# RaptorMai/online-continual-learning

Measured on NVIDIA H100. Metric: replay-step images/sec (ASER+SCR, ResNet18, CIFAR100), higher is better.
Workload: dtype f32

## Files before the change

online-continual-learning_b200/csrc/conv_tcp.cu:

```cuda
#include "conv.cuh"
#include "umma.cuh"

namespace b200ocl {
namespace {

constexpr int TP_THREADS = 32 * 13;
constexpr int TP_LOADER_WARP = 9;
constexpr int TP_PS_MAX = 3;
constexpr int TP_BS_MAX = 6;
constexpr int TP_CONSUMER_WARPS = 8;

using umma::mbar_expect_tx;
using umma::bulk_g2s;

struct TileGeom {
  int wp, pp;
  int tiles_m;
  int prow;
  int pbytes;
};
__host__ __device__ inline TileGeom tile_geom(int N, int H, int W) {
  TileGeom g;
  g.wp = W + 2;
  g.pp = (H + 2) * (W + 2);
  const long last = (long)(N - 1) * g.pp + (long)(H - 1) * g.wp + (W - 1);
  g.tiles_m = (int)(last / 128) + 1;
  g.prow = 128 + 2 * g.wp + 2;
  g.pbytes = (g.prow * 128 + 1023) / 1024 * 1024;
  return g;
}

template <int NT, int KS>
__device__ __forceinline__ void issue_tap(float (&d)[NT / 2], uint64_t dAh, uint64_t dAl, uint64_t dBh, uint64_t dBl) {
  umma::fence();
#pragma unroll
  for (int k = 0; k < KS; ++k) {
    const uint64_t adv = (uint64_t)(k * 2);
    umma::mma_tf32_ss<NT>(d, dAh + adv, dBh + adv, k > 0 ? 1u : 0u);
    umma::mma_tf32_ss<NT>(d, dAh + adv, dBl + adv, 1u);
    umma::mma_tf32_ss<NT>(d, dAl + adv, dBh + adv, 1u);
  }
  umma::commit();
  umma::wait<0>();
  umma::fence_regs(d);
}

template <int NT>
__global__ void __launch_bounds__(TP_THREADS, 1) conv_tcp_kernel(ConvArgs a) {
  constexpr int B_BLOCK = 2 * NT * 32;
  constexpr int R = NT / 2;
  extern __shared__ __align__(1024) unsigned char smem_raw[];
  unsigned char* patch0 = smem_raw;
  __shared__ __align__(8) uint64_t pfull[TP_PS_MAX], pempty[TP_PS_MAX], bfull[9], bempty[TP_BS_MAX];
  __shared__ int s_fail;
  __shared__ float s_coef[3 * 80];

  const int tid = threadIdx.x, warp = tid >> 5;
  const int bn = a.tp_bn;
  const int n0 = blockIdx.y * bn;
  const int slices = a.tp_slices;
  const TileGeom G = tile_geom(a.N, a.Hin, a.Win);
  const int PS = a.tp_ps, BS = a.tp_bs;
  float* sB = reinterpret_cast<float*>(smem_raw + (size_t)PS * 2 * G.pbytes);
  const bool resident = (slices == 1 && NT == 32);
  const int b_slots = resident ? 9 : BS;
  float* s_acc = sB + (size_t)b_slots * B_BLOCK;

  if (tid == 0) {
    for (int i = 0; i < TP_PS_MAX; ++i) {
      umma::mbar_init(&pfull[i], 128);
      umma::mbar_init(&pempty[i], TP_CONSUMER_WARPS);
    }
    for (int i = 0; i < 9; ++i) umma::mbar_init(&bfull[i], 1);
    for (int i = 0; i < TP_BS_MAX; ++i) umma::mbar_init(&bempty[i], TP_CONSUMER_WARPS);
    umma::fence_mbar_init();
    s_fail = 0;
  }
  __syncthreads();
  const float* wimg = a.w_tp + (size_t)blockIdx.y * slices * 9 * B_BLOCK;

  if (warp >= TP_LOADER_WARP) {
    const int lt = tid - 32 * TP_LOADER_WARP;
    int pc = 0;
    for (int tile = blockIdx.x; tile < a.tp_tiles; tile += gridDim.x) {
      for (int sl = 0; sl < slices; ++sl, ++pc) {
        const int ch_valid = min(32, a.CK - sl * 32);
        const int nch = 2 * ((ch_valid + 7) / 8);
        const int ch = lt & 7, r0 = lt >> 3;
        const int nrow = G.prow;
        const bool ch_live = ch < nch, ch_real = ch * 4 < ch_valid;
        float4 v[TP_LD_MAX];
        int img, yp, xp;
        {
          const int sp = tile * 128 + r0;
          img = sp / G.pp;
          const int rem = sp - img * G.pp;
          yp = rem / G.wp;
          xp = rem - yp * G.wp;
        }
        const int hp = a.Hin + 2;
#pragma unroll
        for (int i = 0; i < TP_LD_MAX; ++i) {
          v[i] = make_float4(0.f, 0.f, 0.f, 0.f);
          const int ri = r0 + 16 * i;
          if (ch_real && ri < nrow) {
            const int y = yp - 1, x = xp - 1;
            if (img < a.N && (unsigned)y < (unsigned)a.Hin && (unsigned)x < (unsigned)a.Win)
              v[i] = __ldg(reinterpret_cast<const float4*>(a.in + ((size_t)(img * a.Hin + y) * a.Win + x) * a.CK + sl * 32) + ch);
          }
          xp += 16;
          while (xp >= G.wp) {
            xp -= G.wp;
            if (++yp == hp) {
              yp = 0;
              ++img;
            }
          }
        }
        const int ps = pc % PS;
        if (!umma::mbar_wait(&pempty[ps], (uint32_t)(((pc / PS) & 1) ^ 1))) s_fail = 1;
        float* ph = reinterpret_cast<float*>(patch0 + (size_t)ps * 2 * G.pbytes);
        float* pl = ph + G.pbytes / 4;
        if (ch_live) {
#pragma unroll
          for (int i = 0; i < TP_LD_MAX; ++i) {
            const int ri = r0 + 16 * i;
            if (ri < nrow) {
              float4 h, l;
              umma::split_tf32(v[i].x, h.x, l.x); umma::split_tf32(v[i].y, h.y, l.y);
              umma::split_tf32(v[i].z, h.z, l.z); umma::split_tf32(v[i].w, h.w, l.w);
              const int off = umma::sw128_offset_f32(ri, ch);
              *reinterpret_cast<float4*>(ph + off) = h;
              *reinterpret_cast<float4*>(pl + off) = l;
            }
          }
        }
        umma::fence_proxy_async_smem();
        umma::mbar_arrive(&pfull[ps]);
      }
    }
  } else if (warp == TP_LOADER_WARP - 1) {
    const uint32_t bytes = (uint32_t)(B_BLOCK * sizeof(float));
    if (resident) {
      if (umma::elect_one_sync()) {
        for (int b = 0; b < 9; ++b) {
          mbar_expect_tx(&bfull[b], bytes);
          bulk_g2s(sB + (size_t)b * B_BLOCK, wimg + (size_t)b * B_BLOCK, bytes, &bfull[b]);
        }
      }
    } else {
      int q = 0;
      for (int tile = blockIdx.x; tile < a.tp_tiles; tile += gridDim.x)
        for (int sl = 0; sl < slices; ++sl)
          for (int tap = 0; tap < 9; ++tap, ++q) {
            const int bs = q % BS;
            if (!umma::mbar_wait(&bempty[bs], (uint32_t)(((q / BS) & 1) ^ 1))) s_fail = 1;
            if (umma::elect_one_sync()) {
              mbar_expect_tx(&bfull[bs], bytes);
              bulk_g2s(sB + (size_t)bs * B_BLOCK, wimg + (size_t)(sl * 9 + tap) * B_BLOCK, bytes, &bfull[bs]);
            }
            __syncwarp();
          }
    }
  } else {
    const int g = warp >> 2, wt = tid & 127;
    const int et = tid;
    const bool epi = tid < 128;
    const bool lane0 = (tid & 31) == 0;
    auto esync = []() { asm volatile("bar.sync 1, 128;\n" ::); };
    auto csync = []() { asm volatile("bar.sync 2, 256;\n" ::); };
    const uint64_t dA0 = umma::make_smem_desc_sw128(umma::smem_u32(patch0) + (uint32_t)(g * 64 * 128));
    const uint64_t dB0 = umma::make_smem_desc_sw128(umma::smem_u32(sB));
    const uint32_t A_LO = (uint32_t)G.pbytes >> 4;
    const uint32_t A_STAGE = (uint32_t)(2 * G.pbytes) >> 4;
    constexpr uint32_t B_LO = (NT * 128) >> 4;
    constexpr uint32_t B_SLOT = (B_BLOCK * 4) >> 4;
    if (epi && a.mode == CONV_EVAL) {
      for (int c = et; c < bn; c += 128) {
        const float inv = 1.0f / sqrtf(a.rvar[n0 + c] + a.eps);
        s_coef[c] = a.rmean[n0 + c];
        s_coef[80 + c] = inv * a.gamma[n0 + c];
        s_coef[160 + c] = a.beta[n0 + c];
      }
      esync();
    }
    int pc = 0, q = 0;
    bool b_ready = false;
    for (int tile = blockIdx.x; tile < a.tp_tiles; tile += gridDim.x) {
      float accf[R];
#pragma unroll
      for (int i = 0; i < R; ++i) accf[i] = 0.f;
      for (int sl = 0; sl < slices; ++sl, ++pc) {
        const int ps = pc % PS;
        const int ksteps = (min(32, a.CK - sl * 32) + 7) / 8;
        if (!umma::mbar_wait(&pfull[ps], (uint32_t)((pc / PS) & 1))) s_fail = 1;
        const uint64_t dAs = dA0 + (uint64_t)(ps * A_STAGE);
#pragma unroll 1
        for (int tap = 0; tap < 9; ++tap, ++q) {
          const int kh = tap / 3, kw = tap - 3 * kh;
          const int b = resident ? tap : q % BS;
          if (!(resident && b_ready))
            if (!umma::mbar_wait(&bfull[b], resident ? 0u : (uint32_t)((q / BS) & 1))) s_fail = 1;
          const uint64_t dAh = dAs + (uint64_t)((kh * G.wp + kw) * 8);
          const uint64_t dAl = dAh + A_LO;
          const uint64_t dBh = dB0 + (uint64_t)(b * B_SLOT);
          const uint64_t dBl = dBh + B_LO;
          float tmp[R];
          switch (ksteps) {
            case 1: issue_tap<NT, 1>(tmp, dAh, dAl, dBh, dBl); break;
            case 2: issue_tap<NT, 2>(tmp, dAh, dAl, dBh, dBl); break;
            case 3: issue_tap<NT, 3>(tmp, dAh, dAl, dBh, dBl); break;
            default: issue_tap<NT, 4>(tmp, dAh, dAl, dBh, dBl); break;
          }
#pragma unroll
          for (int i = 0; i < R; ++i) accf[i] += tmp[i];
          if (!resident && lane0) umma::mbar_arrive(&bempty[b]);
        }
        b_ready = true;
        if (lane0) umma::mbar_arrive(&pempty[ps]);
      }
      csync();
#pragma unroll
      for (int i = 0; i < R; ++i) s_acc[(64 * g + umma::frag_row(wt, i)) * (NT + 1) + umma::frag_col(wt, i)] = accf[i];
      csync();
      if (!epi) continue;
      const int sp = tile * 128 + et;
      const int img = sp / G.pp, rem = sp - img * G.pp;
      const int y = rem / G.wp, x = rem - y * G.wp;
      const bool valid = img < a.N && y < a.Hin && x < a.Win;
      const size_t m = ((size_t)img * a.Hin + y) * a.Win + x;
      float acc[NT], pre[NT];
#pragma unroll
      for (int c = 0; c < NT; ++c) {
        acc[c] = 0.f;
        pre[c] = 0.f;
      }
      {
        const float* src = nullptr;
        if (valid && a.mode == CONV_EVAL && a.residual) src = a.residual + m * a.CN + n0;
        if (valid && a.mode == CONV_ACCUM) src = a.out + m * a.CN + n0;
        if (src) {
#pragma unroll
          for (int c0 = 0; c0 < NT; c0 += 4) {
            if (c0 >= bn) break;
            const float4 v = *reinterpret_cast<const float4*>(src + c0);
            pre[c0] = v.x; pre[c0 + 1] = v.y; pre[c0 + 2] = v.z; pre[c0 + 3] = v.w;
          }
        }
      }
#pragma unroll
      for (int c = 0; c < NT; ++c) acc[c] = s_acc[et * (NT + 1) + c];
      if (a.mode == CONV_EVAL) {
        if (valid) {
          float* o = a.out + m * a.CN + n0;
#pragma unroll
          for (int c0 = 0; c0 < NT; c0 += 4) {
            if (c0 >= bn) break;
            float rr[4];
#pragma unroll
            for (int j = 0; j < 4; ++j) {
              rr[j] = (acc[c0 + j] - s_coef[c0 + j]) * s_coef[80 + c0 + j] + s_coef[160 + c0 + j];
              rr[j] += pre[c0 + j];
              if (a.relu) rr[j] = fmaxf(rr[j], 0.f);
            }
            *reinterpret_cast<float4*>(o + c0) = make_float4(rr[0], rr[1], rr[2], rr[3]);
          }
        }
      } else if (valid) {
        float* o = a.out + m * a.CN + n0;
#pragma unroll
        for (int c0 = 0; c0 < NT; c0 += 4) {
          if (c0 >= bn) break;
          *reinterpret_cast<float4*>(o + c0) = make_float4(acc[c0] + pre[c0], acc[c0 + 1] + pre[c0 + 1],
                                                           acc[c0 + 2] + pre[c0 + 2], acc[c0 + 3] + pre[c0 + 3]);
        }
      }
    }
  }
  __syncthreads();
  if (s_fail && tid == 0) a.out[(size_t)n0] = __int_as_float(0x7fc00000);
}

template <int NT>
size_t tcp_smem_bytes(const TileGeom& G, int slices, int ps, int bs) {
  const int b_slots = (slices == 1 && NT == 32) ? 9 : bs;
  return (size_t)ps * 2 * G.pbytes + (size_t)b_slots * 2 * NT * 32 * sizeof(float) +
         (size_t)128 * (NT + 1) * sizeof(float) + 1024;
}

template <int NT>
int launch_tcp(ConvArgs a, cudaStream_t stream) {
  const TileGeom G = tile_geom(a.N, a.Hin, a.Win);
  const size_t limit = 227 * 1024 - 4096
                       - (size_t)128 * (a.tp_bn + 1) * sizeof(float);
  a.tp_ps = 3; a.tp_bs = 6;
  if (tcp_smem_bytes<NT>(G, a.tp_slices, a.tp_ps, a.tp_bs) > limit) a.tp_bs = 4;
  if (tcp_smem_bytes<NT>(G, a.tp_slices, a.tp_ps, a.tp_bs) > limit) { a.tp_ps = 2; a.tp_bs = 6; }
  const size_t smem = tcp_smem_bytes<NT>(G, a.tp_slices, a.tp_ps, a.tp_bs);
  B200OCL_CUDA(raise_smem_limit<conv_tcp_kernel<NT>>(smem));
  a.tp_tiles = G.tiles_m;
  const int n_tiles = a.CN / a.tp_bn;
  int gx = sm_count() / n_tiles;
  if (gx < 1) gx = 1;
  if (gx > G.tiles_m) gx = G.tiles_m;
  const int rounds = (G.tiles_m + gx - 1) / gx;
  gx = (G.tiles_m + rounds - 1) / rounds;
  B200OCL_PROF("conv_tcp",
               2.0 * a.M * (double)a.CN * a.CK * 9.0, stream);
  conv_tcp_kernel<NT><<<dim3(gx, n_tiles), TP_THREADS, smem, stream>>>(a);
  B200OCL_LAUNCHED();
  return B200OCL_OK;
}

}

bool conv_tcp_eligible(const ConvArgs& a) {
  if (a.mode == CONV_TRAIN || !a.w_tp || a.transposed || a.CK % 4 != 0) return false;
  if (a.ks != 3 || a.pad != 1 || a.stride != 1 || a.Hout != a.Hin || a.Wout != a.Win) return false;
  if (!tcp_strip_fits(a.Win)) return false;
  if ((long)a.N * (a.Hin + 2) * (a.Win + 2) > 2000000000L) return false;
  if (a.tp_bn <= 0 || a.tp_bn > 40 || a.CN % a.tp_bn != 0) return false;
  return true;
}

int launch_conv_tcp(const ConvArgs& a, cudaStream_t stream) {
  if (a.tp_bn <= 20) return launch_tcp<32>(a, stream);
  return launch_tcp<48>(a, stream);
}

}
```

online-continual-learning_b200/csrc/umma.cuh:

```cuda
#pragma once
#include <stdint.h>

namespace b200ocl {
namespace umma {

__device__ __forceinline__ uint32_t smem_u32(const void* p) {
  return static_cast<uint32_t>(__cvta_generic_to_shared(p));
}

__device__ __forceinline__ int sw128_offset_f32(int row, int chunk16) {
  return (row >> 3) * 256 + (row & 7) * 32 + ((chunk16 ^ (row & 7)) << 2);
}

__device__ __forceinline__ int frag_row(int t, int i) { return ((t >> 5) << 4) + ((t & 31) >> 2) + ((i & 2) << 2); }
__device__ __forceinline__ int frag_col(int t, int i) { return ((i >> 2) << 3) + ((t & 3) << 1) + (i & 1); }

__device__ __forceinline__ uint64_t make_smem_desc_sw128(uint32_t smem_addr) {
  uint64_t d = 0;
  d |= (uint64_t)((smem_addr >> 4) & 0x3FFF);
  d |= (uint64_t)1 << 16;
  d |= (uint64_t)((1024 >> 4) & 0x3FFF) << 32;
  d |= (uint64_t)1 << 62;
  return d;
}

__device__ __forceinline__ void fence() { asm volatile("wgmma.fence.sync.aligned;\n" ::: "memory"); }
__device__ __forceinline__ void commit() { asm volatile("wgmma.commit_group.sync.aligned;\n" ::: "memory"); }
template <int N>
__device__ __forceinline__ void wait() { asm volatile("wgmma.wait_group.sync.aligned %0;\n" ::"n"(N) : "memory"); }
template <int R>
__device__ __forceinline__ void fence_regs(float (&d)[R]) {
#pragma unroll
  for (int i = 0; i < R; ++i) asm volatile("" : "+f"(d[i])::"memory");
}
__device__ __forceinline__ void fence_proxy_async_smem() { asm volatile("fence.proxy.async.shared::cta;\n" ::); }

__device__ __forceinline__ void mbar_init(uint64_t* bar, uint32_t count) {
  asm volatile("mbarrier.init.shared::cta.b64 [%0], %1;\n" ::"r"(smem_u32(bar)), "r"(count));
}
__device__ __forceinline__ void fence_mbar_init() { asm volatile("fence.mbarrier_init.release.cluster;\n" ::); }
__device__ __forceinline__ bool mbar_wait(uint64_t* bar, uint32_t parity, uint32_t max_spins = (1u << 24)) {
  const uint32_t addr = smem_u32(bar);
#pragma unroll 1
  for (uint32_t i = 0; i < max_spins; ++i) {
    uint32_t done;
    asm volatile(
        "{\n\t.reg .pred p;\n\t"
        "mbarrier.try_wait.parity.shared::cta.b64 p, [%1], %2;\n\t"
        "selp.u32 %0, 1, 0, p;\n\t}\n"
        : "=r"(done)
        : "r"(addr), "r"(parity)
        : "memory");
    if (done) return true;
  }
  return false;
}
__device__ __forceinline__ void mbar_arrive(uint64_t* bar) {
  asm volatile("mbarrier.arrive.shared::cta.b64 _, [%0];\n" ::"r"(smem_u32(bar)) : "memory");
}

__device__ __forceinline__ void mbar_expect_tx(uint64_t* bar, uint32_t bytes) {
  asm volatile("mbarrier.arrive.expect_tx.shared::cta.b64 _, [%0], %1;\n" ::"r"(smem_u32(bar)), "r"(bytes)
               : "memory");
}
__device__ __forceinline__ void bulk_g2s(void* smem_dst, const void* gmem_src, uint32_t bytes, uint64_t* bar) {
  asm volatile(
      "cp.async.bulk.shared::cluster.global.mbarrier::complete_tx::bytes [%0], [%1], %2, [%3];\n" ::"r"(
          smem_u32(smem_dst)),
      "l"(gmem_src), "r"(bytes), "r"(smem_u32(bar))
      : "memory");
}

__device__ __forceinline__ bool elect_one_sync() {
  uint32_t pred;
  asm volatile(
      "{\n\t.reg .pred P;\n\t"
      "elect.sync _|P, 0xffffffff;\n\t"
      "selp.u32 %0, 1, 0, P;\n\t}\n"
      : "=r"(pred));
  return pred != 0;
}

template <int N>
__device__ __forceinline__ void mma_tf32_ss(float (&d)[N / 2], uint64_t desc_a, uint64_t desc_b, uint32_t accumulate);
template <int N>
__device__ __forceinline__ void mma_tf32_rs(float (&d)[N / 2], const uint32_t (&a)[4], uint64_t desc_b, uint32_t accumulate);

template <>
__device__ __forceinline__ void mma_tf32_ss<16>(float (&d)[8], uint64_t desc_a, uint64_t desc_b, uint32_t accumulate) {
  asm volatile(
      "{\n\t.reg .pred p;\n\t"
      "setp.ne.b32 p, %10, 0;\n\t"
      "wgmma.mma_async.sync.aligned.m64n16k8.f32.tf32.tf32 {%0,%1,%2,%3,%4,%5,%6,%7}, %8, %9, p, 1, 1;\n\t}\n"
      : "+f"(d[0]), "+f"(d[1]), "+f"(d[2]), "+f"(d[3]), "+f"(d[4]), "+f"(d[5]), "+f"(d[6]), "+f"(d[7])
      : "l"(desc_a), "l"(desc_b), "r"(accumulate));
}

template <>
__device__ __forceinline__ void mma_tf32_ss<32>(float (&d)[16], uint64_t desc_a, uint64_t desc_b, uint32_t accumulate) {
  asm volatile(
      "{\n\t.reg .pred p;\n\t"
      "setp.ne.b32 p, %18, 0;\n\t"
      "wgmma.mma_async.sync.aligned.m64n32k8.f32.tf32.tf32 {%0,%1,%2,%3,%4,%5,%6,%7,%8,%9,%10,%11,%12,%13,%14,%15}, %16, %17, p, 1, 1;\n\t}\n"
      : "+f"(d[0]), "+f"(d[1]), "+f"(d[2]), "+f"(d[3]), "+f"(d[4]), "+f"(d[5]), "+f"(d[6]), "+f"(d[7]), "+f"(d[8]), "+f"(d[9]), "+f"(d[10]), "+f"(d[11]), "+f"(d[12]), "+f"(d[13]), "+f"(d[14]), "+f"(d[15])
      : "l"(desc_a), "l"(desc_b), "r"(accumulate));
}

template <>
__device__ __forceinline__ void mma_tf32_ss<48>(float (&d)[24], uint64_t desc_a, uint64_t desc_b, uint32_t accumulate) {
  asm volatile(
      "{\n\t.reg .pred p;\n\t"
      "setp.ne.b32 p, %26, 0;\n\t"
      "wgmma.mma_async.sync.aligned.m64n48k8.f32.tf32.tf32 {%0,%1,%2,%3,%4,%5,%6,%7,%8,%9,%10,%11,%12,%13,%14,%15,%16,%17,%18,%19,%20,%21,%22,%23}, %24, %25, p, 1, 1;\n\t}\n"
      : "+f"(d[0]), "+f"(d[1]), "+f"(d[2]), "+f"(d[3]), "+f"(d[4]), "+f"(d[5]), "+f"(d[6]), "+f"(d[7]), "+f"(d[8]), "+f"(d[9]), "+f"(d[10]), "+f"(d[11]), "+f"(d[12]), "+f"(d[13]), "+f"(d[14]), "+f"(d[15]), "+f"(d[16]), "+f"(d[17]), "+f"(d[18]), "+f"(d[19]), "+f"(d[20]), "+f"(d[21]), "+f"(d[22]), "+f"(d[23])
      : "l"(desc_a), "l"(desc_b), "r"(accumulate));
}

template <>
__device__ __forceinline__ void mma_tf32_ss<80>(float (&d)[40], uint64_t desc_a, uint64_t desc_b, uint32_t accumulate) {
  asm volatile(
      "{\n\t.reg .pred p;\n\t"
      "setp.ne.b32 p, %42, 0;\n\t"
      "wgmma.mma_async.sync.aligned.m64n80k8.f32.tf32.tf32 {%0,%1,%2,%3,%4,%5,%6,%7,%8,%9,%10,%11,%12,%13,%14,%15,%16,%17,%18,%19,%20,%21,%22,%23,%24,%25,%26,%27,%28,%29,%30,%31,%32,%33,%34,%35,%36,%37,%38,%39}, %40, %41, p, 1, 1;\n\t}\n"
      : "+f"(d[0]), "+f"(d[1]), "+f"(d[2]), "+f"(d[3]), "+f"(d[4]), "+f"(d[5]), "+f"(d[6]), "+f"(d[7]), "+f"(d[8]), "+f"(d[9]), "+f"(d[10]), "+f"(d[11]), "+f"(d[12]), "+f"(d[13]), "+f"(d[14]), "+f"(d[15]), "+f"(d[16]), "+f"(d[17]), "+f"(d[18]), "+f"(d[19]), "+f"(d[20]), "+f"(d[21]), "+f"(d[22]), "+f"(d[23]), "+f"(d[24]), "+f"(d[25]), "+f"(d[26]), "+f"(d[27]), "+f"(d[28]), "+f"(d[29]), "+f"(d[30]), "+f"(d[31]), "+f"(d[32]), "+f"(d[33]), "+f"(d[34]), "+f"(d[35]), "+f"(d[36]), "+f"(d[37]), "+f"(d[38]), "+f"(d[39])
      : "l"(desc_a), "l"(desc_b), "r"(accumulate));
}

template <>
__device__ __forceinline__ void mma_tf32_rs<32>(float (&d)[16], const uint32_t (&a)[4], uint64_t desc_b, uint32_t accumulate) {
  asm volatile(
      "{\n\t.reg .pred p;\n\t"
      "setp.ne.b32 p, %21, 0;\n\t"
      "wgmma.mma_async.sync.aligned.m64n32k8.f32.tf32.tf32 {%0,%1,%2,%3,%4,%5,%6,%7,%8,%9,%10,%11,%12,%13,%14,%15}, {%16,%17,%18,%19}, %20, p, 1, 1;\n\t}\n"
      : "+f"(d[0]), "+f"(d[1]), "+f"(d[2]), "+f"(d[3]), "+f"(d[4]), "+f"(d[5]), "+f"(d[6]), "+f"(d[7]), "+f"(d[8]), "+f"(d[9]), "+f"(d[10]), "+f"(d[11]), "+f"(d[12]), "+f"(d[13]), "+f"(d[14]), "+f"(d[15])
      : "r"(a[0]), "r"(a[1]), "r"(a[2]), "r"(a[3]), "l"(desc_b), "r"(accumulate));
}

__device__ __forceinline__ float round_tf32(float x) {
  uint32_t r;
  asm("cvt.rna.tf32.f32 %0, %1;\n" : "=r"(r) : "f"(x));
  return __uint_as_float(r);
}
__device__ __forceinline__ void split_tf32(float x, float& hi, float& lo) {
  hi = round_tf32(x);
  lo = x - hi;
}

}
}
```

Baseline: 2042.

## Double-buffer wgmma tap accumulators and split epilogue across both warpgroups

Tensor-core work for each conv tap now goes into one of two alternating register fragments. The next tap is issued before waiting on the previous one (wait<1>), so the wgmma issue no longer fully serializes with the accumulation into the running sum. The epilogue now uses all 256 consumer threads, each handling half the channels of a row, with per-warpgroup barriers instead of a 128-thread epilogue group. The smem budget no longer reserves the accumulator staging area up front, so B stages default to 4. The extra fragment raises register pressure, and mma_tf32_ss_first is only specialized for NT=32/48, so an NT=80 instantiation would fail to compile.

New measurement: 2097 (median of 6 runs). 2.7% higher.

```diff
diff --git a/online-continual-learning_b200/csrc/conv_tcp.cu b/online-continual-learning_b200/csrc/conv_tcp.cu
--- a/online-continual-learning_b200/csrc/conv_tcp.cu
+++ b/online-continual-learning_b200/csrc/conv_tcp.cu
@@ -36,13 +36,12 @@
 #pragma unroll
   for (int k = 0; k < KS; ++k) {
     const uint64_t adv = (uint64_t)(k * 2);
-    umma::mma_tf32_ss<NT>(d, dAh + adv, dBh + adv, k > 0 ? 1u : 0u);
+    if (k == 0) umma::mma_tf32_ss_first<NT>(d, dAh, dBh);
+    else umma::mma_tf32_ss<NT>(d, dAh + adv, dBh + adv, 1u);
     umma::mma_tf32_ss<NT>(d, dAh + adv, dBl + adv, 1u);
     umma::mma_tf32_ss<NT>(d, dAl + adv, dBh + adv, 1u);
   }
   umma::commit();
-  umma::wait<0>();
-  umma::fence_regs(d);
 }
 
 template <int NT>
@@ -163,103 +162,144 @@
           }
     }
   } else {
+    constexpr int EC = NT / 2;
     const int g = warp >> 2, wt = tid & 127;
-    const int et = tid;
-    const bool epi = tid < 128;
     const bool lane0 = (tid & 31) == 0;
-    auto esync = []() { asm volatile("bar.sync 1, 128;\n" ::); };
-    auto csync = []() { asm volatile("bar.sync 2, 256;\n" ::); };
+    auto csync = []() { asm volatile("bar.sync 1, 256;\n" ::); };
+    auto wgsync = [g]() {
+      if (g == 0) asm volatile("bar.sync 2, 128;\n" ::);
+      else asm volatile("bar.sync 3, 128;\n" ::);
+    };
     const uint64_t dA0 = umma::make_smem_desc_sw128(umma::smem_u32(patch0) + (uint32_t)(g * 64 * 128));
     const uint64_t dB0 = umma::make_smem_desc_sw128(umma::smem_u32(sB));
     const uint32_t A_LO = (uint32_t)G.pbytes >> 4;
     const uint32_t A_STAGE = (uint32_t)(2 * G.pbytes) >> 4;
     constexpr uint32_t B_LO = (NT * 128) >> 4;
     constexpr uint32_t B_SLOT = (B_BLOCK * 4) >> 4;
-    if (epi && a.mode == CONV_EVAL) {
-      for (int c = et; c < bn; c += 128) {
+    if (a.mode == CONV_EVAL) {
+      for (int c = tid; c < bn; c += 256) {
         const float inv = 1.0f / sqrtf(a.rvar[n0 + c] + a.eps);
         s_coef[c] = a.rmean[n0 + c];
         s_coef[80 + c] = inv * a.gamma[n0 + c];
         s_coef[160 + c] = a.beta[n0 + c];
       }
-      esync();
-    }
-    int pc = 0, q = 0;
+      csync();
+    }
+    const int taps = 9 * slices;
+    int i_ps = 0, i_pph = 0, i_b = 0, i_bph = 0, i_sl = 0, i_tap = 0;
+    int r_ps = 0, r_b = 0, r_tap = 0;
     bool b_ready = false;
     for (int tile = blockIdx.x; tile < a.tp_tiles; tile += gridDim.x) {
-      float accf[R];
+      float accf[R], f0[R], f1[R];
 #pragma unroll
       for (int i = 0; i < R; ++i) accf[i] = 0.f;
-      for (int sl = 0; sl < slices; ++sl, ++pc) {
-        const int ps = pc % PS;
-        const int ksteps = (min(32, a.CK - sl * 32) + 7) / 8;
-        if (!umma::mbar_wait(&pfull[ps], (uint32_t)((pc / PS) & 1))) s_fail = 1;
-        const uint64_t dAs = dA0 + (uint64_t)(ps * A_STAGE);
+      const bool b_wait = !(resident && b_ready);
+      uint64_t dAs = 0;
+      int ksteps = 0;
+      auto issue = [&](float (&d)[R]) {
+        if (i_tap == 0) {
+          if (!umma::mbar_wait(&pfull[i_ps], (uint32_t)i_pph)) s_fail = 1;
+          dAs = dA0 + (uint64_t)(i_ps * A_STAGE);
+          ksteps = (min(32, a.CK - i_sl * 32) + 7) / 8;
+        }
+        const int kh = i_tap / 3, kw = i_tap - 3 * kh;
+        const int b = i_b;
+        if (b_wait && !umma::mbar_wait(&bfull[b], (uint32_t)i_bph)) s_fail = 1;
+        const uint64_t dAh = dAs + (uint64_t)((kh * G.wp + kw) * 8);
+        const uint64_t dAl = dAh + A_LO;
+        const uint64_t dBh = dB0 + (uint64_t)(b * B_SLOT);
+        const uint64_t dBl = dBh + B_LO;
+        switch (ksteps) {
+          case 1: issue_tap<NT, 1>(d, dAh, dAl, dBh, dBl); break;
+          case 2: issue_tap<NT, 2>(d, dAh, dAl, dBh, dBl); break;
+          case 3: issue_tap<NT, 3>(d, dAh, dAl, dBh, dBl); break;
+          default: issue_tap<NT, 4>(d, dAh, dAl, dBh, dBl); break;
+        }
+        if (++i_b == b_slots) { i_b = 0; i_bph ^= 1; }
+        if (++i_tap == 9) {
+          i_tap = 0;
+          ++i_sl;
+          if (++i_ps == PS) { i_ps = 0; i_pph ^= 1; }
+        }
+      };
+      auto retire = [&](float (&d)[R]) {
+        umma::fence_regs(d);
+#pragma unroll
+        for (int i = 0; i < R; ++i) accf[i] += d[i];
+        if (!resident && lane0) umma::mbar_arrive(&bempty[r_b]);
+        if (++r_b == b_slots) r_b = 0;
+        if (++r_tap == 9) {
+          r_tap = 0;
+          if (lane0) umma::mbar_arrive(&pempty[r_ps]);
+          if (++r_ps == PS) r_ps = 0;
+        }
+      };
+      issue(f0);
+      int t = 1;
 #pragma unroll 1
-        for (int tap = 0; tap < 9; ++tap, ++q) {
-          const int kh = tap / 3, kw = tap - 3 * kh;
-          const int b = resident ? tap : q % BS;
-          if (!(resident && b_ready))
-            if (!umma::mbar_wait(&bfull[b], resident ? 0u : (uint32_t)((q / BS) & 1))) s_fail = 1;
-          const uint64_t dAh = dAs + (uint64_t)((kh * G.wp + kw) * 8);
-          const uint64_t dAl = dAh + A_LO;
-          const uint64_t dBh = dB0 + (uint64_t)(b * B_SLOT);
-          const uint64_t dBl = dBh + B_LO;
-          float tmp[R];
-          switch (ksteps) {
-            case 1: issue_tap<NT, 1>(tmp, dAh, dAl, dBh, dBl); break;
-            case 2: issue_tap<NT, 2>(tmp, dAh, dAl, dBh, dBl); break;
-            case 3: issue_tap<NT, 3>(tmp, dAh, dAl, dBh, dBl); break;
-            default: issue_tap<NT, 4>(tmp, dAh, dAl, dBh, dBl); break;
-          }
-#pragma unroll
-          for (int i = 0; i < R; ++i) accf[i] += tmp[i];
-          if (!resident && lane0) umma::mbar_arrive(&bempty[b]);
-        }
-        b_ready = true;
-        if (lane0) umma::mbar_arrive(&pempty[ps]);
-      }
-      csync();
+      do {
+        issue(f1);
+        umma::wait<1>();
+        retire(f0);
+        issue(f0);
+        umma::wait<1>();
+        retire(f1);
+        t += 2;
+      } while (t + 1 < taps);
+      if (t < taps) {
+        issue(f1);
+        umma::wait<1>();
+        retire(f0);
+        umma::wait<0>();
+        retire(f1);
+      } else {
+        umma::wait<0>();
+        retire(f0);
+      }
+      i_sl = 0;
+      b_ready = true;
+      wgsync();
 #pragma unroll
       for (int i = 0; i < R; ++i) s_acc[(64 * g + umma::frag_row(wt, i)) * (NT + 1) + umma::frag_col(wt, i)] = accf[i];
-      csync();
-      if (!epi) continue;
-      const int sp = tile * 128 + et;
+      wgsync();
+      const int row = 64 * g + (wt >> 1), c1 = (wt & 1) * EC;
+      const int sp = tile * 128 + row;
       const int img = sp / G.pp, rem = sp - img * G.pp;
       const int y = rem / G.wp, x = rem - y * G.wp;
       const bool valid = img < a.N && y < a.Hin && x < a.Win;
       const size_t m = ((size_t)img * a.Hin + y) * a.Win + x;
-      float acc[NT], pre[NT];
-#pragma unroll
-      for (int c = 0; c < NT; ++c) {
+      float acc[EC], pre[EC];
+#pragma unroll
+      for (int c = 0; c < EC; ++c) {
         acc[c] = 0.f;
         pre[c] = 0.f;
       }
       {
         const float* src = nullptr;
-        if (valid && a.mode == CONV_EVAL && a.residual) src = a.residual + m * a.CN + n0;
-        if (valid && a.mode == CONV_ACCUM) src = a.out + m * a.CN + n0;
+        if (valid && a.mode == CONV_EVAL && a.residual) src = a.residual + m * a.CN + n0 + c1;
+        if (valid && a.mode == CONV_ACCUM) src = a.out + m * a.CN + n0 + c1;
         if (src) {
 #pragma unroll
-          for (int c0 = 0; c0 < NT; c0 += 4) {
-            if (c0 >= bn) break;
+          for (int c0 = 0; c0 < EC; c0 += 4) {
+            if (c1 + c0 >= bn) break;
             const float4 v = *reinterpret_cast<const float4*>(src + c0);
             pre[c0] = v.x; pre[c0 + 1] = v.y; pre[c0 + 2] = v.z; pre[c0 + 3] = v.w;
           }
         }
       }
 #pragma unroll
-      for (int c = 0; c < NT; ++c) acc[c] = s_acc[et * (NT + 1) + c];
+      for (int c = 0; c < EC; ++c) acc[c] = s_acc[row * (NT + 1) + c1 + c];
       if (a.mode == CONV_EVAL) {
         if (valid) {
-          float* o = a.out + m * a.CN + n0;
-#pragma unroll
-          for (int c0 = 0; c0 < NT; c0 += 4) {
-            if (c0 >= bn) break;
+          float* o = a.out + m * a.CN + n0 + c1;
+          const float* k = s_coef + c1;
+#pragma unroll
+          for (int c0 = 0; c0 < EC; c0 += 4) {
+            if (c1 + c0 >= bn) break;
             float rr[4];
 #pragma unroll
             for (int j = 0; j < 4; ++j) {
-              rr[j] = (acc[c0 + j] - s_coef[c0 + j]) * s_coef[80 + c0 + j] + s_coef[160 + c0 + j];
+              rr[j] = (acc[c0 + j] - k[c0 + j]) * k[80 + c0 + j] + k[160 + c0 + j];
               rr[j] += pre[c0 + j];
               if (a.relu) rr[j] = fmaxf(rr[j], 0.f);
             }
@@ -267,10 +307,10 @@
           }
         }
       } else if (valid) {
-        float* o = a.out + m * a.CN + n0;
-#pragma unroll
-        for (int c0 = 0; c0 < NT; c0 += 4) {
-          if (c0 >= bn) break;
+        float* o = a.out + m * a.CN + n0 + c1;
+#pragma unroll
+        for (int c0 = 0; c0 < EC; c0 += 4) {
+          if (c1 + c0 >= bn) break;
           *reinterpret_cast<float4*>(o + c0) = make_float4(acc[c0] + pre[c0], acc[c0 + 1] + pre[c0 + 1],
                                                            acc[c0 + 2] + pre[c0 + 2], acc[c0 + 3] + pre[c0 + 3]);
         }
@@ -291,10 +331,8 @@
 template <int NT>
 int launch_tcp(ConvArgs a, cudaStream_t stream) {
   const TileGeom G = tile_geom(a.N, a.Hin, a.Win);
-  const size_t limit = 227 * 1024 - 4096
-                       - (size_t)128 * (a.tp_bn + 1) * sizeof(float);
-  a.tp_ps = 3; a.tp_bs = 6;
-  if (tcp_smem_bytes<NT>(G, a.tp_slices, a.tp_ps, a.tp_bs) > limit) a.tp_bs = 4;
+  const size_t limit = 227 * 1024 - 4096;
+  a.tp_ps = 3; a.tp_bs = 4;
   if (tcp_smem_bytes<NT>(G, a.tp_slices, a.tp_ps, a.tp_bs) > limit) { a.tp_ps = 2; a.tp_bs = 6; }
   const size_t smem = tcp_smem_bytes<NT>(G, a.tp_slices, a.tp_ps, a.tp_bs);
   B200OCL_CUDA(raise_smem_limit<conv_tcp_kernel<NT>>(smem));
diff --git a/online-continual-learning_b200/csrc/umma.cuh b/online-continual-learning_b200/csrc/umma.cuh
--- a/online-continual-learning_b200/csrc/umma.cuh
+++ b/online-continual-learning_b200/csrc/umma.cuh
@@ -116,6 +116,29 @@
       : "l"(desc_a), "l"(desc_b), "r"(accumulate));
 }
 
+template <int N>
+__device__ __forceinline__ void mma_tf32_ss_first(float (&d)[N / 2], uint64_t desc_a, uint64_t desc_b);
+
+template <>
+__device__ __forceinline__ void mma_tf32_ss_first<32>(float (&d)[16], uint64_t desc_a, uint64_t desc_b) {
+  asm volatile(
+      "{\n\t.reg .pred p;\n\t"
+      "setp.ne.b32 p, %18, 0;\n\t"
+      "wgmma.mma_async.sync.aligned.m64n32k8.f32.tf32.tf32 {%0,%1,%2,%3,%4,%5,%6,%7,%8,%9,%10,%11,%12,%13,%14,%15}, %16, %17, p, 1, 1;\n\t}\n"
+      : "=f"(d[0]), "=f"(d[1]), "=f"(d[2]), "=f"(d[3]), "=f"(d[4]), "=f"(d[5]), "=f"(d[6]), "=f"(d[7]), "=f"(d[8]), "=f"(d[9]), "=f"(d[10]), "=f"(d[11]), "=f"(d[12]), "=f"(d[13]), "=f"(d[14]), "=f"(d[15])
+      : "l"(desc_a), "l"(desc_b), "n"(0));
+}
+
+template <>
+__device__ __forceinline__ void mma_tf32_ss_first<48>(float (&d)[24], uint64_t desc_a, uint64_t desc_b) {
+  asm volatile(
+      "{\n\t.reg .pred p;\n\t"
+      "setp.ne.b32 p, %26, 0;\n\t"
+      "wgmma.mma_async.sync.aligned.m64n48k8.f32.tf32.tf32 {%0,%1,%2,%3,%4,%5,%6,%7,%8,%9,%10,%11,%12,%13,%14,%15,%16,%17,%18,%19,%20,%21,%22,%23}, %24, %25, p, 1, 1;\n\t}\n"
+      : "=f"(d[0]), "=f"(d[1]), "=f"(d[2]), "=f"(d[3]), "=f"(d[4]), "=f"(d[5]), "=f"(d[6]), "=f"(d[7]), "=f"(d[8]), "=f"(d[9]), "=f"(d[10]), "=f"(d[11]), "=f"(d[12]), "=f"(d[13]), "=f"(d[14]), "=f"(d[15]), "=f"(d[16]), "=f"(d[17]), "=f"(d[18]), "=f"(d[19]), "=f"(d[20]), "=f"(d[21]), "=f"(d[22]), "=f"(d[23])
+      : "l"(desc_a), "l"(desc_b), "n"(0));
+}
+
 template <>
 __device__ __forceinline__ void mma_tf32_ss<80>(float (&d)[40], uint64_t desc_a, uint64_t desc_b, uint32_t accumulate) {
   asm volatile(
```
